# H263/review-based-recommender

Measured on NVIDIA B200. Metric: DeepCoNN fwd+bwd samples/sec, higher is better.
Workload: dtype bf16

## Files before the change

review-based-recommender_b200/csrc/conv_bwd_tc.cu:

```cuda
#include "rbr_common.cuh"
#include "tc_ptx.cuh"
#include "tma_util.cuh"

namespace rbr {

constexpr int CM_THREADS = 192;
constexpr int CM_STAGES_T = 3;
constexpr int CM_STAGES_W = 3;

struct CmatLayout {
    int64_t V, H, K, E, HJ, HJp, emb_pad, epad4;
    int64_t off_c32, off_chl, off_dw, total;
    int64_t n_chunks, hc;
};
struct CmatChunk { int64_t h_lo, h_n, col_lo, width, base; };
static CmatLayout cmat_layout(int64_t vocab, int64_t emb, int64_t filters, int64_t ksize) {
    CmatLayout l;
    l.V = vocab; l.H = filters; l.K = ksize; l.E = emb;
    l.HJ = filters * ksize;
    l.HJp = cmat_hjp(filters, ksize);
    l.emb_pad = rbr_emb_pad(emb);
    l.epad4 = round_up(emb, 4);
    int64_t off = 0;
    l.off_c32 = off; off += round_up(vocab * l.HJp * 4, 1024);
// ... 165 lines not shown
        hi.x = *reinterpret_cast<const uint32_t*>(&h01); hi.y = *reinterpret_cast<const uint32_t*>(&h23);
        lo.x = *reinterpret_cast<const uint32_t*>(&l01); lo.y = *reinterpret_cast<const uint32_t*>(&l23);
        __nv_bfloat16* row = chl + r * (2 * (int64_t)HJp);
        *reinterpret_cast<uint2*>(row + c) = hi;
        *reinterpret_cast<uint2*>(row + HJp + c) = lo;
    }
}

__device__ __forceinline__ uint64_t umma_desc_mn_sw128(uint32_t addr, uint32_t lbo, uint32_t sbo) {
    return (uint64_t)((addr >> 4) & 0x3FFFu) | ((uint64_t)((lbo >> 4) & 0x3FFFu) << 16) | ((uint64_t)((sbo >> 4) & 0x3FFFu) << 32) |
           (1ull << 46) | (2ull << 61);
}
__device__ __forceinline__ uint32_t umma_idesc_mn(int M, int N) { return umma_idesc(M, N) | (1u << 15) | (1u << 16); }

struct TableGemmArgs {
    int64_t vocab;
    int E, NT, nkb;
    int64_t padding_idx;
    float* table_grad;
    int overwrite;
    int tile0;
};

__global__ void __launch_bounds__(CM_THREADS, 2)
cmat_table_gemm_kernel(const __grid_constant__ CUtensorMap tmA, const __grid_constant__ CUtensorMap tmB, const TableGemmArgs a) {
    extern __shared__ uint8_t smem_raw[];
    const int warp = threadIdx.x >> 5, lane = threadIdx.x & 31;
    const uint32_t raw = smem_u32(smem_raw);
    const uint32_t sbase = (raw + 1023u) & ~1023u;
    uint8_t* smem = smem_raw + (sbase - raw);
    const int b_bytes = a.NT * 128;
    const int stage_bytes = 16384 + b_bytes;
    const uint32_t bars = sbase + CM_STAGES_T * stage_bytes;
    volatile uint32_t* tmem_slot = reinterpret_cast<volatile uint32_t*>(smem + CM_STAGES_T * stage_bytes + 8 * (2 * CM_STAGES_T + 1));
    const int m0 = ((int)blockIdx.x + a.tile0) * 128, n0 = blockIdx.y * a.NT;

    if (threadIdx.x == 0) {
        for (int i = 0; i < CM_STAGES_T; ++i) { mbar_init(bars + 8 * i, 1); mbar_init(bars + 8 * (CM_STAGES_T + i), 1); }
        mbar_init(bars + 16 * CM_STAGES_T, 1);
        fence_barrier_init();
    }
    if (warp == 1) tmem_alloc(smem_u32((const void*)tmem_slot), 256);
    tc_fence_before();
    __syncthreads();
    tc_fence_after();
    const uint32_t tmem_base = *tmem_slot;

    if (warp == 0) {
        if (elect_one()) {
            tma_prefetch_desc(&tmA);
            tma_prefetch_desc(&tmB);
            int stage = 0;
            uint32_t ph = 0;
            for (int kb = 0; kb < a.nkb; ++kb) {
                mbar_wait(bars + 8 * (CM_STAGES_T + stage), ph ^ 1);
                const uint32_t fb = bars + 8 * stage;
                mbar_expect_tx(fb, (uint32_t)stage_bytes);
                const uint32_t dst = sbase + stage * stage_bytes;
                tma_load_2d(dst, &tmA, kb * 64, m0, fb);
                tma_load_2d(dst + 16384, &tmB, kb * 64, n0, fb);
                if (++stage == CM_STAGES_T) { stage = 0; ph ^= 1; }
            }
        }
        __syncwarp();
    } else if (warp == 1) {
        const uint32_t idesc = umma_idesc(128, a.NT);
        int stage = 0;
        uint32_t ph = 0;
        for (int kb = 0; kb < a.nkb; ++kb) {
            mbar_wait(bars + 8 * stage, ph);
            tc_fence_after();
            if (elect_one()) {
                const uint32_t sa = sbase + stage * stage_bytes;
                const uint64_t ad = umma_desc_sw128(sa), bd = umma_desc_sw128(sa + 16384);
#pragma unroll
                for (int ks = 0; ks < 4; ++ks)
                    umma_bf16(tmem_base, ad + (uint64_t)(ks * 2), bd + (uint64_t)(ks * 2), idesc, (uint32_t)((kb | ks) != 0));
                umma_commit(bars + 8 * (CM_STAGES_T + stage));
                if (kb == a.nkb - 1) umma_commit(bars + 16 * CM_STAGES_T);
            }
            __syncwarp();
            if (++stage == CM_STAGES_T) { stage = 0; ph ^= 1; }
        }
    } else {
        const int quad = warp & 3;
        const int64_t row = (int64_t)m0 + quad * 32 + lane;
        const bool in_range = row < a.vocab;
        const bool pad_row = row == a.padding_idx;
        const bool live = in_range && (a.overwrite || !pad_row);
        const float keep = pad_row ? 0.f : 1.f;
        float* dst_row = a.table_grad + row * a.E;
        mbar_wait(bars + 16 * CM_STAGES_T, 0);
        tc_fence_after();
        const uint32_t taddr = tmem_base + ((uint32_t)(quad * 32) << 16);
        for (int c0 = 0; c0 < a.NT; c0 += 16) {
            uint32_t v[16];
            tmem_ld16(taddr + (uint32_t)c0, v);
            tmem_ld_wait();
            if (live) {
#pragma unroll
                for (int q = 0; q < 4; ++q) {
                    const int col = n0 + c0 + q * 4;
                    if (col + 3 < a.E) {
                        float4* p = reinterpret_cast<float4*>(dst_row + col);
                        float4 o = make_float4(0.f, 0.f, 0.f, 0.f);
                        if (!a.overwrite) o = *p;
                        o.x += keep * __uint_as_float(v[4 * q]); o.y += keep * __uint_as_float(v[4 * q + 1]);
                        o.z += keep * __uint_as_float(v[4 * q + 2]); o.w += keep * __uint_as_float(v[4 * q + 3]);
                        __stcs(p, o);
                    }
                }
            }
        }
    }
    tc_fence_before();
    __syncthreads();
    if (warp == 1) tmem_dealloc(tmem_base, 256);
}

struct WeightGemmArgs {
    int64_t vocab;
    int E, epad4, HJ, HJp, nch;
    int n_tb, ksplit;
    float* dw_hke;
};

__global__ void __launch_bounds__(CM_THREADS, 1)
cmat_weight_gemm_kernel(const __grid_constant__ CUtensorMap tmA, const __grid_constant__ CUtensorMap tmX, const WeightGemmArgs a) {
    extern __shared__ uint8_t smem_raw[];
    const int warp = threadIdx.x >> 5, lane = threadIdx.x & 31;
    const uint32_t raw = smem_u32(smem_raw);
    const uint32_t sbase = (raw + 1023u) & ~1023u;
    uint8_t* smem = smem_raw + (sbase - raw);
    const int stage_bytes = (2 + a.nch) * 8192;
    const uint32_t bars = sbase + CM_STAGES_W * stage_bytes;
    volatile uint32_t* tmem_slot = reinterpret_cast<volatile uint32_t*>(smem + CM_STAGES_W * stage_bytes + 8 * (2 * CM_STAGES_W + 1));
    const int m0 = blockIdx.x * 128;
    const int split = blockIdx.y;
    const int n_mine = (a.n_tb - split + a.ksplit - 1) / a.ksplit;
    const uint32_t tmem_cols = a.nch * 64 <= 256 ? 256u : 512u;

    if (threadIdx.x == 0) {
        for (int i = 0; i < CM_STAGES_W; ++i) { mbar_init(bars + 8 * i, 1); mbar_init(bars + 8 * (CM_STAGES_W + i), 1); }
        mbar_init(bars + 16 * CM_STAGES_W, 1);
        fence_barrier_init();
    }
    if (warp == 1) tmem_alloc(smem_u32((const void*)tmem_slot), tmem_cols);
    tc_fence_before();
    __syncthreads();
    tc_fence_after();
    const uint32_t tmem_base = *tmem_slot;

    if (n_mine > 0) {
        if (warp == 0) {
            if (elect_one()) {
                tma_prefetch_desc(&tmA);
                tma_prefetch_desc(&tmX);
                int stage = 0;
                uint32_t ph = 0;
                for (int i = 0; i < n_mine; ++i) {
                    const int row = (split + i * a.ksplit) * 64;
                    mbar_wait(bars + 8 * (CM_STAGES_W + stage), ph ^ 1);
                    const uint32_t fb = bars + 8 * stage;
                    mbar_expect_tx(fb, (uint32_t)stage_bytes);
                    const uint32_t dst = sbase + stage * stage_bytes;
                    tma_load_2d(dst, &tmA, m0, row, fb);
                    tma_load_2d(dst + 8192, &tmA, m0 + 64, row, fb);
                    for (int c = 0; c < a.nch; ++c) tma_load_2d(dst + 16384 + c * 8192, &tmX, c * 64, row, fb);
                    if (++stage == CM_STAGES_W) { stage = 0; ph ^= 1; }
                }
            }
            __syncwarp();
        } else if (warp == 1) {
            const int g0 = a.nch <= 4 ? a.nch : (a.nch + 1) / 2, g1 = a.nch - g0;
            const uint32_t idesc0 = umma_idesc_mn(128, g0 * 64), idesc1 = g1 ? umma_idesc_mn(128, g1 * 64) : 0u;
            int stage = 0;
            uint32_t ph = 0;
            for (int i = 0; i < n_mine; ++i) {
                mbar_wait(bars + 8 * stage, ph);
                tc_fence_after();
                if (elect_one()) {
                    const uint32_t sa = sbase + stage * stage_bytes, sb = sa + 16384;
#pragma unroll
                    for (int ks = 0; ks < 4; ++ks) {
                        const uint64_t ad = umma_desc_mn_sw128(sa + ks * 2048, 8192, 1024);
                        umma_bf16(tmem_base, ad, umma_desc_mn_sw128(sb + ks * 2048, 8192, 1024), idesc0, (uint32_t)((i | ks) != 0));
                        if (g1)
                            umma_bf16(tmem_base + (uint32_t)(g0 * 64), ad, umma_desc_mn_sw128(sb + g0 * 8192 + ks * 2048, 8192, 1024), idesc1,
                                      (uint32_t)((i | ks) != 0));
                    }
                    umma_commit(bars + 8 * (CM_STAGES_W + stage));
                    if (i == n_mine - 1) umma_commit(bars + 16 * CM_STAGES_W);
                }
                __syncwarp();
                if (++stage == CM_STAGES_W) { stage = 0; ph ^= 1; }
            }
        } else {
            const int quad = warp & 3;
            const int gm = m0 + quad * 32 + lane;
            const int hj = gm >= a.HJp ? gm - a.HJp : gm;
            const bool live = hj < a.HJ;
            float* dst_row = a.dw_hke + (int64_t)hj * a.epad4;
            mbar_wait(bars + 16 * CM_STAGES_W, 0);
            tc_fence_after();
            const uint32_t taddr = tmem_base + ((uint32_t)(quad * 32) << 16);
            for (int c0 = 0; c0 < a.nch * 64; c0 += 16) {
                uint32_t v[16];
                tmem_ld16(taddr + (uint32_t)c0, v);
                tmem_ld_wait();
                if (live) {
#pragma unroll
                    for (int q = 0; q < 4; ++q) {
                        const int col = c0 + q * 4;
                        if (col + 3 < a.E)
                            atomicAdd(reinterpret_cast<float4*>(dst_row + col),
                                      make_float4(__uint_as_float(v[4 * q]), __uint_as_float(v[4 * q + 1]), __uint_as_float(v[4 * q + 2]),
                                                  __uint_as_float(v[4 * q + 3])));
                    }
// ... 8 lines not shown

__global__ void cmat_unpack_kernel(float* __restrict__ dw_hke, int H, int E, int K, int epad4, float* __restrict__ wgrad) {
    const int64_t total = (int64_t)H * K * epad4;
    const int64_t stride = (int64_t)gridDim.x * blockDim.x;
    for (int64_t q = (int64_t)blockIdx.x * blockDim.x + threadIdx.x; q < total; q += stride) {
        const int e = (int)(q % epad4);
        const int hj = (int)(q / epad4);
        const float v = dw_hke[q];
        if (v != 0.f) {
            dw_hke[q] = 0.f;
            if (e < E) atomicAdd(wgrad + ((int64_t)(hj / K) * E + e) * K + (hj % K), v);
        }
    }
}

constexpr int CM_SMEM_T_MAX = 116 * 1024;
constexpr int CM_SMEM_W_MAX = 227 * 1024;
struct CmatSmem { int table, weight; };
static CmatSmem cmat_smem(int64_t emb) {
    int64_t NT, tiles;
    cmat_ntile(emb, &NT, &tiles);
    const int64_t nch = rbr_emb_pad(emb) / 64;
    CmatSmem s;
    s.table = CM_STAGES_T * (16384 + (int)NT * 128) + 8 * (2 * CM_STAGES_T + 1) + 16 + 1024;
    s.weight = CM_STAGES_W * (2 + (int)nch) * 8192 + 8 * (2 * CM_STAGES_W + 1) + 16 + 1024;
    return s;
}

static bool cmat_shape_ok(int64_t vocab, int64_t emb, int64_t filters, int64_t ksize) {
    if (vocab < 1 || vocab >= (1ll << 31) || emb < 4 || emb % 4 != 0 || emb > 512 || filters < 1 || ksize < 1 || ksize > 8) return false;
    if (filters > 1024) return false;
    const CmatSmem sm = cmat_smem(emb);
    if (sm.table > CM_SMEM_T_MAX || sm.weight > CM_SMEM_W_MAX) return false;
    const int64_t hjp = cmat_hjp(filters, ksize);
    if (hjp > 4096) return false;
    return vocab * hjp * 4 <= (3ll << 30);
}

}

using namespace rbr;

extern "C" int rbr_conv_bwd_cmat_supported(int64_t vocab, int64_t emb, int64_t filters, int64_t ksize) {
    return cmat_shape_ok(vocab, emb, filters, ksize) && tensor_map_encoder() != nullptr ? 1 : 0;
}
// ... 124 lines not shown
        for (int64_t c = (chunk < 0 ? 0 : chunk); c < (chunk < 0 ? l.n_chunks : chunk + 1); ++c) {
            const CmatChunk k = cmat_chunk(l, c);
            const int64_t total = vocab * (k.width / 4);
            int64_t blocks = (total + 255) / 256;
            if (blocks > 148 * 16) blocks = 148 * 16;
            cmat_split_kernel<<<(unsigned)blocks, 256, 0, s>>>(reinterpret_cast<const float4*>(c32 + k.base), vocab, (int)k.width, (int)k.col_lo,
                                                               (int)l.HJp, chl);
            RBR_LAUNCH_CHECK("cmat_split_kernel");
        }
    }
    if (what & 2) {
        RBR_REQUIRE(table_grad, RBR_EINVAL, "conv_bwd_cmat_finish: table part needs table_grad");
        RBR_REQUIRE((uintptr_t)table_grad % 16 == 0, RBR_EINVAL, "conv_bwd_cmat_finish: table_grad must be 16-byte aligned");
        CUtensorMap tmA, tmB;
        RBR_REQUIRE(make_tmap_bf16_2d(&tmA, chl, (uint64_t)(2 * l.HJp), (uint64_t)vocab, (uint64_t)(2 * l.HJp), 64, 128) &&
                        make_tmap_bf16_2d(&tmB, reinterpret_cast<const char*>(packed) + pl.off_wt2, (uint64_t)(2 * l.HJp),
                                          (uint64_t)(pl.NT * pl.n_tiles), (uint64_t)(2 * l.HJp), 64, (uint32_t)pl.NT),
                    RBR_ECUDA, "conv_bwd_cmat_finish: cuTensorMapEncodeTiled failed");
        TableGemmArgs a{};
        a.vocab = vocab; a.E = (int)emb; a.NT = (int)pl.NT; a.nkb = (int)(2 * l.HJp / 64); a.padding_idx = padding_idx;
        a.table_grad = table_grad;
        a.overwrite = (what & 8) ? 1 : 0;
        if (row_lo == 0 && row_hi == 0) row_hi = vocab;
        RBR_REQUIRE(row_lo >= 0 && row_lo < row_hi && row_hi <= vocab && row_lo % 128 == 0 && (row_hi % 128 == 0 || row_hi == vocab), RBR_EINVAL,
                    "conv_bwd_cmat_finish: the table row range must be cut on multiples of 128 rows");
        a.tile0 = (int)(row_lo / 128);
        const int smem = cmat_smem(emb).table;
        static bool attr = false;
        if (!attr) {
            RBR_CUDA(cudaFuncSetAttribute(cmat_table_gemm_kernel, cudaFuncAttributeMaxDynamicSharedMemorySize, CM_SMEM_T_MAX));
            attr = true;
        }
        RBR_REQUIRE(smem <= CM_SMEM_T_MAX, RBR_EUNSUPPORTED, "conv_bwd_cmat_finish: shared memory");
        dim3 grid((unsigned)((row_hi - row_lo + 127) / 128), (unsigned)pl.n_tiles);
        cmat_table_gemm_kernel<<<grid, CM_THREADS, smem, s>>>(tmA, tmB, a);
        RBR_LAUNCH_CHECK("cmat_table_gemm_kernel");
    }
    if (what & 4) {
        RBR_REQUIRE(weight_grad && shadow_bf16, RBR_EINVAL, "conv_bwd_cmat_finish: weight part needs weight_grad and the bf16 shadow table");
        CUtensorMap tmA, tmX;
        RBR_REQUIRE(make_tmap_bf16_2d(&tmA, chl, (uint64_t)(2 * l.HJp), (uint64_t)vocab, (uint64_t)(2 * l.HJp), 64, 64) &&
                        make_tmap_bf16_2d(&tmX, shadow_bf16, (uint64_t)l.emb_pad, (uint64_t)vocab, (uint64_t)l.emb_pad, 64, 64),
                    RBR_ECUDA, "conv_bwd_cmat_finish: cuTensorMapEncodeTiled failed");
        WeightGemmArgs a{};
        a.vocab = vocab; a.E = (int)emb; a.epad4 = (int)l.epad4; a.HJ = (int)l.HJ; a.HJp = (int)l.HJp; a.nch = (int)(l.emb_pad / 64);
        a.n_tb = (int)((vocab + 63) / 64);
        const int m_tiles = (int)(2 * l.HJp / 128);
        static int sms = 0;
        if (!sms) {
            int dev = 0;
            RBR_CUDA(cudaGetDevice(&dev));
            RBR_CUDA(cudaDeviceGetAttribute(&sms, cudaDevAttrMultiProcessorCount, dev));
        }
        a.ksplit = sms / m_tiles < 1 ? 1 : sms / m_tiles;
        if (a.ksplit > a.n_tb) a.ksplit = a.n_tb;
        a.dw_hke = dw;
        const int smem = cmat_smem(emb).weight;
        static bool attr = false;
        if (!attr) {
            RBR_CUDA(cudaFuncSetAttribute(cmat_weight_gemm_kernel, cudaFuncAttributeMaxDynamicSharedMemorySize, CM_SMEM_W_MAX));
            attr = true;
        }
        RBR_REQUIRE(smem <= CM_SMEM_W_MAX, RBR_EUNSUPPORTED, "conv_bwd_cmat_finish: shared memory");
        dim3 grid((unsigned)m_tiles, (unsigned)a.ksplit);
        cmat_weight_gemm_kernel<<<grid, CM_THREADS, smem, s>>>(tmA, tmX, a);
        RBR_LAUNCH_CHECK("cmat_weight_gemm_kernel");
        const int64_t tot = l.HJ * l.epad4;
        int blocks = (int)((tot + 255) / 256);
        if (blocks > 148 * 4) blocks = 148 * 4;
        cmat_unpack_kernel<<<blocks, 256, 0, s>>>(dw, (int)filters, (int)emb, (int)ksize, (int)l.epad4, weight_grad);
        RBR_LAUNCH_CHECK("cmat_unpack_kernel");
    }
    return RBR_OK;
}
```

review-based-recommender_b200/csrc/embed.cu:

```cuda
#include "rbr_common.cuh"
#include "token_sort.cuh"

namespace rbr {

template <int UNROLL>
__global__ void __launch_bounds__(256) gather_rows_v4_kernel(const float4* __restrict__ table, int64_t vocab, int e4,
                                                             const int64_t* __restrict__ ids, int64_t n_tokens,
                                                             float4* __restrict__ out) {
    const int64_t total = n_tokens * (int64_t)e4;
    const int64_t stride = (int64_t)gridDim.x * blockDim.x;
    int64_t q = (int64_t)blockIdx.x * blockDim.x + threadIdx.x;
    for (; q + (UNROLL - 1) * stride < total; q += UNROLL * stride) {
        float4 v[UNROLL];
        int64_t dst[UNROLL];
#pragma unroll
        for (int u = 0; u < UNROLL; ++u) {
            const int64_t p = q + u * stride;
            const int64_t tok = p / e4;
            const int c = (int)(p - tok * e4);
            const int64_t id = __ldg(ids + tok);
            dst[u] = p;
            if (id >= 0 && id < vocab) {
                v[u] = __ldg(table + id * e4 + c);
            } else {
// ... 119 lines not shown
#pragma unroll
        for (int j = 0; j < 8; ++j) f[j] = (c0 + j < emb) ? __ldg(src + j) : 0.f;
        uint4 pk;
        __nv_bfloat162 t;
        t = __floats2bfloat162_rn(f[0], f[1]); pk.x = *reinterpret_cast<uint32_t*>(&t);
        t = __floats2bfloat162_rn(f[2], f[3]); pk.y = *reinterpret_cast<uint32_t*>(&t);
        t = __floats2bfloat162_rn(f[4], f[5]); pk.z = *reinterpret_cast<uint32_t*>(&t);
        t = __floats2bfloat162_rn(f[6], f[7]); pk.w = *reinterpret_cast<uint32_t*>(&t);
        *reinterpret_cast<uint4*>(shadow + row * emb_pad + c0) = pk;
    }
}

__global__ void conv_pack_kernel(const float* __restrict__ w, int E, int H, int k, int Hpad4, int Epad4, int Epad16, int Npad, int Nb,
                                 int Npad2, int Nb2, float* __restrict__ keh, float* __restrict__ hke,
                                 __nv_bfloat16* __restrict__ umma, __nv_bfloat16* __restrict__ umma2, __nv_bfloat16* __restrict__ hke16,
                                 __nv_bfloat16* __restrict__ wt2, int HJp, int wt2_rows) {
    const int64_t n_keh = (int64_t)k * E * Hpad4;
    const int64_t n_hke = (int64_t)H * k * Epad4;
    const int64_t n_umma = (int64_t)k * Epad16 * Npad;
    const int64_t n_umma2 = (int64_t)k * Epad16 * Npad2;
    const int64_t n_wt2 = (int64_t)wt2_rows * 2 * HJp;
    const int64_t total = n_keh + n_hke + n_umma + n_umma2 + n_wt2;
    const int64_t stride = (int64_t)gridDim.x * blockDim.x;
    for (int64_t q = (int64_t)blockIdx.x * blockDim.x + threadIdx.x; q < total; q += stride) {
        if (q >= n_keh + n_hke + n_umma + n_umma2) {
            const int64_t r = q - (n_keh + n_hke + n_umma + n_umma2);
            const int e = (int)(r / (2 * HJp));
            int c = (int)(r - (int64_t)e * 2 * HJp);
            if (c >= HJp) c -= HJp;
            const int h = c / k, j = c - h * k;
            wt2[r] = __float2bfloat16_rn((e < E && h < H) ? w[((int64_t)h * E + e) * k + j] : 0.f);
        } else if (q < n_keh) {
            const int h = (int)(q % Hpad4);
            const int e = (int)((q / Hpad4) % E);
            const int j = (int)(q / ((int64_t)Hpad4 * E));
            keh[q] = (h < H) ? w[((int64_t)h * E + e) * k + j] : 0.f;
        } else if (q < n_keh + n_hke) {
            const int64_t r = q - n_keh;
            const int e = (int)(r % Epad4);
            const int j = (int)((r / Epad4) % k);
            const int h = (int)(r / ((int64_t)Epad4 * k));
            const float v = (e < E) ? w[((int64_t)h * E + e) * k + j] : 0.f;
            hke[r] = v;
            hke16[r] = __float2bfloat16_rn(v);
        } else if (q >= n_keh + n_hke + n_umma) {
            const int64_t r = q - n_keh - n_hke - n_umma;
// ... 113 lines not shown
}

extern "C" int64_t rbr_conv_pack_bytes(int64_t emb, int64_t filters, int64_t ksize) {
    return pack_layout(emb, filters, ksize).total;
}

extern "C" int rbr_conv_pack(const float* weight, int64_t emb, int64_t filters, int64_t ksize, void* packed, void* stream) {
    RBR_REQUIRE(weight && packed, RBR_EINVAL, "rbr_conv_pack: null pointer");
    RBR_REQUIRE(emb > 0 && filters > 0 && ksize > 0, RBR_EINVAL, "rbr_conv_pack: bad sizes");
    RBR_REQUIRE((uintptr_t)packed % 256 == 0, RBR_EINVAL, "rbr_conv_pack: packed buffer must be 256-byte aligned");
    const PackLayout p = pack_layout(emb, filters, ksize);
    char* base = reinterpret_cast<char*>(packed);
    RBR_CUDA(cudaMemsetAsync(base + p.off_zero, 0, (size_t)(p.off_umma2 - p.off_zero), as_stream(stream)));
    const int64_t npad2 = p.P2 * p.Nb2;
    const int64_t total = ksize * emb * p.Hpad4 + filters * ksize * p.Epad4 + ksize * p.Epad16 * (p.Npad + npad2) +
                          p.NT * p.n_tiles * 2 * p.HJp;
    conv_pack_kernel<<<grid_for(total, 256), 256, 0, as_stream(stream)>>>(
        weight, (int)emb, (int)filters, (int)ksize, (int)p.Hpad4, (int)p.Epad4, (int)p.Epad16, (int)p.Npad, (int)(p.Nb > 0 ? p.Nb : 1),
        (int)npad2, (int)(p.Nb2 > 0 ? p.Nb2 : 2), reinterpret_cast<float*>(base + p.off_keh), reinterpret_cast<float*>(base + p.off_hke),
        reinterpret_cast<__nv_bfloat16*>(base + p.off_umma), reinterpret_cast<__nv_bfloat16*>(base + p.off_umma2),
        reinterpret_cast<__nv_bfloat16*>(base + p.off_hke16), reinterpret_cast<__nv_bfloat16*>(base + p.off_wt2), (int)p.HJp,
        (int)(p.NT * p.n_tiles));
    RBR_LAUNCH_CHECK("conv_pack");
    return RBR_OK;
}

RBR_DEFINE_OOB_ACCESSOR(embed)
```

review-based-recommender_b200/csrc/rbr_common.cuh:

```cuda
#pragma once
#include <cuda_runtime.h>
#include <cuda_bf16.h>
#include <stdint.h>
#include <stdio.h>
#include <stdarg.h>

#include "../../include/rbr_b200.h"

namespace rbr {

void set_error(const char* fmt, ...);
int cuda_fail(cudaError_t e, const char* what);

#define RBR_REQUIRE(cond, code, ...)                    \
    do {                                                \
        if (!(cond)) {                                  \
            rbr::set_error(__VA_ARGS__);                \
            return (code);                              \
        }                                               \
    } while (0)

#define RBR_CUDA(call)                                                   \
    do {                                                                 \
        cudaError_t e__ = (call);                                        \
// ... 26 lines not shown
void tc_pass_split(int64_t E, int64_t H, int64_t K, int64_t* P, int64_t* Nb);
void tc2_pass_split(int64_t E, int64_t H, int64_t K, int64_t* P, int64_t* Nb);
struct PackLayout {
    int64_t E, H, k;
    int64_t P, Nb;
    int64_t P2, Nb2;
    int64_t off_umma2;
    int64_t off_hke16;
    int64_t Hpad4;
    int64_t Epad4;
    int64_t Epad16;
    int64_t Npad;
    int64_t off_keh, off_hke, off_umma, off_zero, total;
    int64_t HJp;
    int64_t NT, n_tiles;
    int64_t off_wt2;
};
__host__ __device__ inline int64_t round_up(int64_t x, int64_t m) { return (x + m - 1) / m * m; }
inline int64_t cmat_hjp(int64_t H, int64_t k) { return round_up(H * k, 64); }
inline void cmat_ntile(int64_t E, int64_t* NT, int64_t* tiles) {
    *NT = E > 128 ? 160 : round_up(E, 16);
    *tiles = (E + *NT - 1) / *NT;
}
inline PackLayout pack_layout(int64_t E, int64_t H, int64_t k) {
    PackLayout p;
    p.E = E; p.H = H; p.k = k;
    p.Hpad4 = round_up(H, 4);
    p.Epad4 = round_up(E, 4);
    p.Epad16 = round_up(E, 16);
    tc_pass_split(E, H, k, &p.P, &p.Nb);
    p.Npad = p.P * p.Nb;
    p.off_keh = 0;
    int64_t b = k * E * p.Hpad4 * 4;
    p.off_hke = round_up(b, 256);
    b = p.off_hke + H * k * p.Epad4 * 4;
    p.off_umma = round_up(b, 256);
    b = p.off_umma + k * p.Epad16 * p.Npad * 2;
    p.off_zero = round_up(b, 256);
    b = p.off_zero + round_up(E, 64) * 2 + 256;
    p.off_umma2 = round_up(b, 256);
    tc2_pass_split(E, H, k, &p.P2, &p.Nb2);
    b = p.off_umma2 + k * p.Epad16 * p.P2 * p.Nb2 * 2;
    p.off_hke16 = round_up(b, 256);
    b = p.off_hke16 + H * k * p.Epad4 * 2;
    p.off_wt2 = round_up(b, 1024);
    p.HJp = cmat_hjp(H, k);
    cmat_ntile(E, &p.NT, &p.n_tiles);
    b = p.off_wt2 + p.NT * p.n_tiles * 2 * p.HJp * 2;
    p.total = round_up(b, 256);
    return p;
}

__device__ __forceinline__ float warp_sum(float v) {
#pragma unroll
    for (int o = 16; o > 0; o >>= 1) v += __shfl_xor_sync(0xffffffffu, v, o);
    return v;
}
__device__ __forceinline__ float warp_max(float v) {
#pragma unroll
    for (int o = 16; o > 0; o >>= 1) v = fmaxf(v, __shfl_xor_sync(0xffffffffu, v, o));
    return v;
}

// ... 36 lines not shown
```

review-based-recommender_b200/csrc/tc_ptx.cuh:

```cuda
#pragma once
#include "rbr_common.cuh"

namespace rbr {

__device__ __forceinline__ uint32_t smem_u32(const void* p) { return (uint32_t)__cvta_generic_to_shared(p); }

__device__ __forceinline__ void mbar_init(uint32_t bar, uint32_t count) {
    asm volatile("mbarrier.init.shared::cta.b64 [%0], %1;" ::"r"(bar), "r"(count));
}
__device__ __forceinline__ void mbar_arrive(uint32_t bar) {
    asm volatile("mbarrier.arrive.shared::cta.b64 _, [%0];" ::"r"(bar) : "memory");
}
__device__ __forceinline__ void mbar_expect_tx(uint32_t bar, uint32_t bytes) {
    asm volatile("mbarrier.arrive.expect_tx.shared::cta.b64 _, [%0], %1;" ::"r"(bar), "r"(bytes) : "memory");
}
__device__ __forceinline__ bool mbar_try_wait(uint32_t bar, uint32_t parity) {
    uint32_t ok;
    asm volatile(
        "{\n\t.reg .pred p;\n\t"
        "mbarrier.try_wait.parity.shared::cta.b64 p, [%1], %2;\n\t"
        "selp.u32 %0, 1, 0, p;\n\t}"
        : "=r"(ok)
        : "r"(bar), "r"(parity)
        : "memory");
// ... 55 lines not shown
}
__device__ __forceinline__ uint32_t umma_idesc(int M, int N) {
    return (1u << 4) | (1u << 7) | (1u << 10) | ((uint32_t)(N >> 3) << 17) | ((uint32_t)(M >> 4) << 24);
}
__device__ __forceinline__ void umma_bf16(uint32_t tmem_d, uint64_t adesc, uint64_t bdesc, uint32_t idesc, uint32_t accumulate) {
    asm volatile(
        "{\n\t.reg .pred p;\n\t"
        "setp.ne.b32 p, %4, 0;\n\t"
        "tcgen05.mma.cta_group::1.kind::f16 [%0], %1, %2, %3, p;\n\t}" ::"r"(tmem_d),
        "l"(adesc), "l"(bdesc), "r"(idesc), "r"(accumulate)
        : "memory");
}
__device__ __forceinline__ void umma_commit(uint32_t bar) {
    asm volatile("tcgen05.commit.cta_group::1.mbarrier::arrive::one.shared::cluster.b64 [%0];" ::"r"(bar) : "memory");
}
__device__ __forceinline__ void tmem_ld16(uint32_t taddr, uint32_t (&v)[16]) {
    asm volatile(
        "tcgen05.ld.sync.aligned.32x32b.x16.b32 {%0,%1,%2,%3,%4,%5,%6,%7,%8,%9,%10,%11,%12,%13,%14,%15}, [%16];"
        : "=r"(v[0]), "=r"(v[1]), "=r"(v[2]), "=r"(v[3]), "=r"(v[4]), "=r"(v[5]), "=r"(v[6]), "=r"(v[7]), "=r"(v[8]), "=r"(v[9]),
          "=r"(v[10]), "=r"(v[11]), "=r"(v[12]), "=r"(v[13]), "=r"(v[14]), "=r"(v[15])
        : "r"(taddr)
        : "memory");
}
__device__ __forceinline__ bool elect_one() {
    uint32_t pred;
    asm volatile(
        "{\n\t.reg .pred p;\n\t"
        "elect.sync _|p, 0xffffffff;\n\t"
        "selp.u32 %0, 1, 0, p;\n\t}"
        : "=r"(pred));
// ... 26 lines not shown
    }
#pragma unroll
    for (int i = 0; i < 16; ++i) {
        const uint32_t b = __ballot_sync(0xffffffffu, (FULL || mine) && (int)v[i] == r[i]);
        if ((lane & 15) == i) { keep_v = (uint32_t)r[i]; keep_b = b; }
    }
}



__device__ __forceinline__ uint32_t cluster_ctarank() {
    uint32_t r;
    asm volatile("mov.u32 %0, %%cluster_ctarank;" : "=r"(r));
    return r;
}
__device__ __forceinline__ void cluster_sync_all() {
    asm volatile("barrier.cluster.arrive.release.aligned;\n\tbarrier.cluster.wait.acquire.aligned;" ::: "memory");
}
__device__ __forceinline__ void mbar_arrive_cluster(uint32_t bar, uint32_t cta) {
    asm volatile(
        "{\n\t.reg .b32 ra;\n\t"
        "mapa.shared::cluster.u32 ra, %0, %1;\n\t"
        "mbarrier.arrive.shared::cluster.b64 _, [ra];\n\t}" ::"r"(bar), "r"(cta)
        : "memory");
}
__device__ __forceinline__ void tmem_alloc2(uint32_t slot_smem, uint32_t cols) {
    asm volatile("tcgen05.alloc.cta_group::2.sync.aligned.shared::cta.b32 [%0], %1;" ::"r"(slot_smem), "r"(cols) : "memory");
    asm volatile("tcgen05.relinquish_alloc_permit.cta_group::2.sync.aligned;" ::: "memory");
}
__device__ __forceinline__ void tmem_dealloc2(uint32_t taddr, uint32_t cols) {
// ... 32 lines not shown
```

review-based-recommender_b200/csrc/tma_util.cuh:

```cuda
#pragma once
#include <cuda.h>

#include "rbr_common.cuh"

namespace rbr {

typedef CUresult (*EncodeTiledFn)(CUtensorMap*, CUtensorMapDataType, cuuint32_t, void*, const cuuint64_t*, const cuuint64_t*,
                                  const cuuint32_t*, const cuuint32_t*, CUtensorMapInterleave, CUtensorMapSwizzle,
                                  CUtensorMapL2promotion, CUtensorMapFloatOOBfill);

inline EncodeTiledFn tensor_map_encoder() {
    static EncodeTiledFn fn = nullptr;
    static bool tried = false;
    if (!tried) {
        tried = true;
        void* f = nullptr;
        cudaDriverEntryPointQueryResult q;
        if (cudaGetDriverEntryPoint("cuTensorMapEncodeTiled", &f, cudaEnableDefault, &q) == cudaSuccess &&
            q == cudaDriverEntryPointSuccess)
            fn = reinterpret_cast<EncodeTiledFn>(f);
        else
            (void)cudaGetLastError();
    }
    return fn;
}

inline bool make_tmap_bf16_2d(CUtensorMap* tm, const void* base, uint64_t cols, uint64_t rows, uint64_t pitch_elems,
                              uint32_t box_cols, uint32_t box_rows) {
    EncodeTiledFn enc = tensor_map_encoder();
    if (!enc) return false;
    cuuint64_t gdim[2] = {(cuuint64_t)cols, (cuuint64_t)rows};
    cuuint64_t gstr[1] = {(cuuint64_t)pitch_elems * 2};
    cuuint32_t box[2] = {box_cols, box_rows};
    cuuint32_t estr[2] = {1, 1};
    return enc(tm, CU_TENSOR_MAP_DATA_TYPE_BFLOAT16, 2, const_cast<void*>(base), gdim, gstr, box, estr, CU_TENSOR_MAP_INTERLEAVE_NONE,
               CU_TENSOR_MAP_SWIZZLE_128B, CU_TENSOR_MAP_L2_PROMOTION_L2_256B, CU_TENSOR_MAP_FLOAT_OOB_FILL_NONE) == CUDA_SUCCESS;
}

__device__ __forceinline__ void tma_load_2d(uint32_t dst, const void* tmap, int col, int row, uint32_t bar) {
    asm volatile(
        "cp.async.bulk.tensor.2d.shared::cluster.global.tile.mbarrier::complete_tx::bytes [%0], [%1, {%2, %3}], [%4];" ::"r"(dst),
        "l"(tmap), "r"(col), "r"(row), "r"(bar)
        : "memory");
}

}
```

Measured before the change: 5.348 million.

## Multicast table-GEMM A tiles across cluster, TMA-store epilogue, split hi/lo weights

Restructures the embedding-table gradient GEMM. The hi and lo halves of the split-bf16 C matrix now load as two A boxes sharing one B tile, multicast across a CTA cluster, and the packed weight copy holding the duplicated B becomes a single non-duplicated one. The epilogue stages results in swizzled shared memory and writes them out with TMA store or reduce-add bulk ops instead of per-thread float4 read-modify-write. The weight GEMM loads hi and lo through separate tensor maps and accumulates both into the same TMEM. This cuts global traffic and scattered stores, at the cost of cluster synchronisation, fewer table pipeline stages and a lower supported maximum embedding size.

```diff
diff --git a/review-based-recommender_b200/csrc/conv_bwd_tc.cu b/review-based-recommender_b200/csrc/conv_bwd_tc.cu
--- a/review-based-recommender_b200/csrc/conv_bwd_tc.cu
+++ b/review-based-recommender_b200/csrc/conv_bwd_tc.cu
@@ -5,8 +5,7 @@
 namespace rbr {
 
 constexpr int CM_THREADS = 192;
-constexpr int CM_STAGES_T = 3;
-constexpr int CM_STAGES_W = 3;
+constexpr int CM_STAGES_T = 2;
 
 struct CmatLayout {
     int64_t V, H, K, E, HJ, HJp, emb_pad, epad4;
@@ -203,35 +202,38 @@
 __device__ __forceinline__ uint32_t umma_idesc_mn(int M, int N) { return umma_idesc(M, N) | (1u << 15) | (1u << 16); }
 
 struct TableGemmArgs {
-    int64_t vocab;
-    int E, NT, nkb;
+    int NT, HJp, nkb;
+    int nbox;
     int64_t padding_idx;
-    float* table_grad;
     int overwrite;
     int tile0;
 };
 
 __global__ void __launch_bounds__(CM_THREADS, 2)
-cmat_table_gemm_kernel(const __grid_constant__ CUtensorMap tmA, const __grid_constant__ CUtensorMap tmB, const TableGemmArgs a) {
+cmat_table_gemm_kernel(const __grid_constant__ CUtensorMap tmA, const __grid_constant__ CUtensorMap tmB, const __grid_constant__ CUtensorMap tmOut,
+                       const TableGemmArgs a) {
     extern __shared__ uint8_t smem_raw[];
     const int warp = threadIdx.x >> 5, lane = threadIdx.x & 31;
     const uint32_t raw = smem_u32(smem_raw);
     const uint32_t sbase = (raw + 1023u) & ~1023u;
     uint8_t* smem = smem_raw + (sbase - raw);
     const int b_bytes = a.NT * 128;
-    const int stage_bytes = 16384 + b_bytes;
+    const int stage_bytes = 2 * 16384 + b_bytes;
     const uint32_t bars = sbase + CM_STAGES_T * stage_bytes;
     volatile uint32_t* tmem_slot = reinterpret_cast<volatile uint32_t*>(smem + CM_STAGES_T * stage_bytes + 8 * (2 * CM_STAGES_T + 1));
     const int m0 = ((int)blockIdx.x + a.tile0) * 128, n0 = blockIdx.y * a.NT;
+    const int ncta = (int)cluster_nctarank();
+    const int rank = (int)cluster_ctarank();
+    const uint16_t cluster_mask = (uint16_t)((1u << ncta) - 1u);
 
     if (threadIdx.x == 0) {
-        for (int i = 0; i < CM_STAGES_T; ++i) { mbar_init(bars + 8 * i, 1); mbar_init(bars + 8 * (CM_STAGES_T + i), 1); }
+        for (int i = 0; i < CM_STAGES_T; ++i) { mbar_init(bars + 8 * i, 1); mbar_init(bars + 8 * (CM_STAGES_T + i), (uint32_t)ncta); }
         mbar_init(bars + 16 * CM_STAGES_T, 1);
         fence_barrier_init();
     }
     if (warp == 1) tmem_alloc(smem_u32((const void*)tmem_slot), 256);
     tc_fence_before();
-    __syncthreads();
+    cluster_sync_all();
     tc_fence_after();
     const uint32_t tmem_base = *tmem_slot;
 
@@ -246,8 +248,15 @@
                 const uint32_t fb = bars + 8 * stage;
                 mbar_expect_tx(fb, (uint32_t)stage_bytes);
                 const uint32_t dst = sbase + stage * stage_bytes;
-                tma_load_2d(dst, &tmA, kb * 64, m0, fb);
-                tma_load_2d(dst + 16384, &tmB, kb * 64, n0, fb);
+                for (int b = rank; b < 2; b += ncta) {
+                    if (ncta == 1) tma_load_2d(dst + b * 16384, &tmA, b * a.HJp + kb * 64, m0, fb);
+                    else tma_load_2d_mc(dst + b * 16384, &tmA, b * a.HJp + kb * 64, m0, fb, cluster_mask);
+                }
+                tma_load_2d(dst + 2 * 16384, &tmB, kb * 64, n0, fb);
+                if (++stage == CM_STAGES_T) { stage = 0; ph ^= 1; }
+            }
+            for (int i = 0; i < CM_STAGES_T; ++i) {
+                mbar_wait(bars + 8 * (CM_STAGES_T + stage), ph ^ 1);
                 if (++stage == CM_STAGES_T) { stage = 0; ph ^= 1; }
             }
         }
@@ -261,11 +270,16 @@
             tc_fence_after();
             if (elect_one()) {
                 const uint32_t sa = sbase + stage * stage_bytes;
-                const uint64_t ad = umma_desc_sw128(sa), bd = umma_desc_sw128(sa + 16384);
-#pragma unroll
-                for (int ks = 0; ks < 4; ++ks)
-                    umma_bf16(tmem_base, ad + (uint64_t)(ks * 2), bd + (uint64_t)(ks * 2), idesc, (uint32_t)((kb | ks) != 0));
-                umma_commit(bars + 8 * (CM_STAGES_T + stage));
+                const uint64_t bd = umma_desc_sw128(sa + 2 * 16384);
+#pragma unroll
+                for (int b = 0; b < 2; ++b) {
+                    const uint64_t ad = umma_desc_sw128(sa + b * 16384);
+#pragma unroll
+                    for (int ks = 0; ks < 4; ++ks)
+                        umma_bf16(tmem_base, ad + (uint64_t)(ks * 2), bd + (uint64_t)(ks * 2), idesc, (uint32_t)((kb | b | ks) != 0));
+                }
+                if (ncta == 1) umma_commit(bars + 8 * (CM_STAGES_T + stage));
+                else umma_commit_mc(bars + 8 * (CM_STAGES_T + stage), cluster_mask);
                 if (kb == a.nkb - 1) umma_commit(bars + 16 * CM_STAGES_T);
             }
             __syncwarp();
@@ -273,65 +287,70 @@
         }
     } else {
         const int quad = warp & 3;
-        const int64_t row = (int64_t)m0 + quad * 32 + lane;
-        const bool in_range = row < a.vocab;
-        const bool pad_row = row == a.padding_idx;
-        const bool live = in_range && (a.overwrite || !pad_row);
-        const float keep = pad_row ? 0.f : 1.f;
-        float* dst_row = a.table_grad + row * a.E;
+        const int row0 = m0 + quad * 32;
+        const bool pad_row = (int64_t)(row0 + lane) == a.padding_idx;
+        const uint32_t out = sbase + (uint32_t)(quad * a.nbox) * 4096u;
         mbar_wait(bars + 16 * CM_STAGES_T, 0);
         tc_fence_after();
         const uint32_t taddr = tmem_base + ((uint32_t)(quad * 32) << 16);
-        for (int c0 = 0; c0 < a.NT; c0 += 16) {
+        for (int c0 = 0; c0 < a.nbox * 32; c0 += 16) {
             uint32_t v[16];
             tmem_ld16(taddr + (uint32_t)c0, v);
             tmem_ld_wait();
-            if (live) {
-#pragma unroll
-                for (int q = 0; q < 4; ++q) {
-                    const int col = n0 + c0 + q * 4;
-                    if (col + 3 < a.E) {
-                        float4* p = reinterpret_cast<float4*>(dst_row + col);
-                        float4 o = make_float4(0.f, 0.f, 0.f, 0.f);
-                        if (!a.overwrite) o = *p;
-                        o.x += keep * __uint_as_float(v[4 * q]); o.y += keep * __uint_as_float(v[4 * q + 1]);
-                        o.z += keep * __uint_as_float(v[4 * q + 2]); o.w += keep * __uint_as_float(v[4 * q + 3]);
-                        __stcs(p, o);
-                    }
-                }
-            }
-        }
+            const uint32_t line = out + (uint32_t)(c0 >> 5) * 4096u + (uint32_t)lane * 128u;
+#pragma unroll
+            for (int q = 0; q < 4; ++q) {
+                const uint32_t chunk = (uint32_t)(((c0 & 31) >> 2) + q);
+                st_shared_v4(line + ((chunk ^ (uint32_t)(lane & 7)) << 4), pad_row ? 0u : v[4 * q], pad_row ? 0u : v[4 * q + 1],
+                             pad_row ? 0u : v[4 * q + 2], pad_row ? 0u : v[4 * q + 3]);
+            }
+        }
+        fence_proxy_async();
+        __syncwarp();
+        if (lane == 0) {
+            const uint64_t policy = l2_policy_evict_first();
+            for (int b = 0; b < a.nbox; ++b) {
+                if (a.overwrite) tma_store_2d(&tmOut, out + (uint32_t)b * 4096u, n0 + b * 32, row0, policy);
+                else tma_reduce_add_2d(&tmOut, out + (uint32_t)b * 4096u, n0 + b * 32, row0, policy);
+            }
+            bulk_commit_group();
+            bulk_wait_group_read0();
+        }
+        __syncwarp();
     }
     tc_fence_before();
-    __syncthreads();
+    cluster_sync_all();
     if (warp == 1) tmem_dealloc(tmem_base, 256);
 }
 
 struct WeightGemmArgs {
     int64_t vocab;
-    int E, epad4, HJ, HJp, nch;
+    int E, epad4, HJ, nch;
+    int stages;
     int n_tb, ksplit;
     float* dw_hke;
 };
 
 __global__ void __launch_bounds__(CM_THREADS, 1)
-cmat_weight_gemm_kernel(const __grid_constant__ CUtensorMap tmA, const __grid_constant__ CUtensorMap tmX, const WeightGemmArgs a) {
+cmat_weight_gemm_kernel(const __grid_constant__ CUtensorMap tmHi, const __grid_constant__ CUtensorMap tmLo, const __grid_constant__ CUtensorMap tmX,
+                        const WeightGemmArgs a) {
     extern __shared__ uint8_t smem_raw[];
     const int warp = threadIdx.x >> 5, lane = threadIdx.x & 31;
     const uint32_t raw = smem_u32(smem_raw);
     const uint32_t sbase = (raw + 1023u) & ~1023u;
     uint8_t* smem = smem_raw + (sbase - raw);
-    const int stage_bytes = (2 + a.nch) * 8192;
-    const uint32_t bars = sbase + CM_STAGES_W * stage_bytes;
-    volatile uint32_t* tmem_slot = reinterpret_cast<volatile uint32_t*>(smem + CM_STAGES_W * stage_bytes + 8 * (2 * CM_STAGES_W + 1));
+    const int S = a.stages;
+    const int stage_bytes = (4 + a.nch) * 8192;
+    const uint32_t bars = sbase + S * stage_bytes;
+    volatile uint32_t* tmem_slot = reinterpret_cast<volatile uint32_t*>(smem + S * stage_bytes + 8 * (2 * S + 1));
     const int m0 = blockIdx.x * 128;
     const int split = blockIdx.y;
     const int n_mine = (a.n_tb - split + a.ksplit - 1) / a.ksplit;
     const uint32_t tmem_cols = a.nch * 64 <= 256 ? 256u : 512u;
 
     if (threadIdx.x == 0) {
-        for (int i = 0; i < CM_STAGES_W; ++i) { mbar_init(bars + 8 * i, 1); mbar_init(bars + 8 * (CM_STAGES_W + i), 1); }
-        mbar_init(bars + 16 * CM_STAGES_W, 1);
+        for (int i = 0; i < S; ++i) { mbar_init(bars + 8 * i, 1); mbar_init(bars + 8 * (S + i), 1); }
+        mbar_init(bars + 16 * S, 1);
         fence_barrier_init();
     }
     if (warp == 1) tmem_alloc(smem_u32((const void*)tmem_slot), tmem_cols);
@@ -343,20 +362,23 @@
     if (n_mine > 0) {
         if (warp == 0) {
             if (elect_one()) {
-                tma_prefetch_desc(&tmA);
+                tma_prefetch_desc(&tmHi);
+                tma_prefetch_desc(&tmLo);
                 tma_prefetch_desc(&tmX);
                 int stage = 0;
                 uint32_t ph = 0;
                 for (int i = 0; i < n_mine; ++i) {
                     const int row = (split + i * a.ksplit) * 64;
-                    mbar_wait(bars + 8 * (CM_STAGES_W + stage), ph ^ 1);
+                    mbar_wait(bars + 8 * (S + stage), ph ^ 1);
                     const uint32_t fb = bars + 8 * stage;
                     mbar_expect_tx(fb, (uint32_t)stage_bytes);
                     const uint32_t dst = sbase + stage * stage_bytes;
-                    tma_load_2d(dst, &tmA, m0, row, fb);
-                    tma_load_2d(dst + 8192, &tmA, m0 + 64, row, fb);
-                    for (int c = 0; c < a.nch; ++c) tma_load_2d(dst + 16384 + c * 8192, &tmX, c * 64, row, fb);
-                    if (++stage == CM_STAGES_W) { stage = 0; ph ^= 1; }
+                    tma_load_2d(dst, &tmHi, m0, row, fb);
+                    tma_load_2d(dst + 8192, &tmHi, m0 + 64, row, fb);
+                    tma_load_2d(dst + 2 * 8192, &tmLo, m0, row, fb);
+                    tma_load_2d(dst + 3 * 8192, &tmLo, m0 + 64, row, fb);
+                    for (int c = 0; c < a.nch; ++c) tma_load_2d(dst + (4 + c) * 8192, &tmX, c * 64, row, fb);
+                    if (++stage == S) { stage = 0; ph ^= 1; }
                 }
             }
             __syncwarp();
@@ -369,28 +391,31 @@
                 mbar_wait(bars + 8 * stage, ph);
                 tc_fence_after();
                 if (elect_one()) {
-                    const uint32_t sa = sbase + stage * stage_bytes, sb = sa + 16384;
+                    const uint32_t sa = sbase + stage * stage_bytes, sb = sa + 4 * 8192;
 #pragma unroll
                     for (int ks = 0; ks < 4; ++ks) {
-                        const uint64_t ad = umma_desc_mn_sw128(sa + ks * 2048, 8192, 1024);
-                        umma_bf16(tmem_base, ad, umma_desc_mn_sw128(sb + ks * 2048, 8192, 1024), idesc0, (uint32_t)((i | ks) != 0));
-                        if (g1)
-                            umma_bf16(tmem_base + (uint32_t)(g0 * 64), ad, umma_desc_mn_sw128(sb + g0 * 8192 + ks * 2048, 8192, 1024), idesc1,
-                                      (uint32_t)((i | ks) != 0));
+                        const uint64_t bd0 = umma_desc_mn_sw128(sb + ks * 2048, 8192, 1024);
+                        const uint64_t bd1 = umma_desc_mn_sw128(sb + g0 * 8192 + ks * 2048, 8192, 1024);
+#pragma unroll
+                        for (int h = 0; h < 2; ++h) {
+                            const uint64_t ad = umma_desc_mn_sw128(sa + h * 16384 + ks * 2048, 8192, 1024);
+                            const uint32_t acc = (uint32_t)((i | ks | h) != 0);
+                            umma_bf16(tmem_base, ad, bd0, idesc0, acc);
+                            if (g1) umma_bf16(tmem_base + (uint32_t)(g0 * 64), ad, bd1, idesc1, acc);
+                        }
                     }
-                    umma_commit(bars + 8 * (CM_STAGES_W + stage));
-                    if (i == n_mine - 1) umma_commit(bars + 16 * CM_STAGES_W);
+                    umma_commit(bars + 8 * (S + stage));
+                    if (i == n_mine - 1) umma_commit(bars + 16 * S);
                 }
                 __syncwarp();
-                if (++stage == CM_STAGES_W) { stage = 0; ph ^= 1; }
+                if (++stage == S) { stage = 0; ph ^= 1; }
             }
         } else {
             const int quad = warp & 3;
-            const int gm = m0 + quad * 32 + lane;
-            const int hj = gm >= a.HJp ? gm - a.HJp : gm;
+            const int hj = m0 + quad * 32 + lane;
             const bool live = hj < a.HJ;
             float* dst_row = a.dw_hke + (int64_t)hj * a.epad4;
-            mbar_wait(bars + 16 * CM_STAGES_W, 0);
+            mbar_wait(bars + 16 * S, 0);
             tc_fence_after();
             const uint32_t taddr = tmem_base + ((uint32_t)(quad * 32) << 16);
             for (int c0 = 0; c0 < a.nch * 64; c0 += 16) {
@@ -429,21 +454,23 @@
     }
 }
 
-constexpr int CM_SMEM_T_MAX = 116 * 1024;
+constexpr int CM_SMEM_T_MAX = 112 * 1024;
 constexpr int CM_SMEM_W_MAX = 227 * 1024;
+static int cmat_w_smem(int64_t nch, int stages) { return stages * (4 + (int)nch) * 8192 + 8 * (2 * stages + 1) + 16 + 1024; }
+static int cmat_w_stages(int64_t nch) { return cmat_w_smem(nch, 3) <= CM_SMEM_W_MAX ? 3 : 2; }
 struct CmatSmem { int table, weight; };
 static CmatSmem cmat_smem(int64_t emb) {
     int64_t NT, tiles;
     cmat_ntile(emb, &NT, &tiles);
     const int64_t nch = rbr_emb_pad(emb) / 64;
     CmatSmem s;
-    s.table = CM_STAGES_T * (16384 + (int)NT * 128) + 8 * (2 * CM_STAGES_T + 1) + 16 + 1024;
-    s.weight = CM_STAGES_W * (2 + (int)nch) * 8192 + 8 * (2 * CM_STAGES_W + 1) + 16 + 1024;
+    s.table = CM_STAGES_T * (2 * 16384 + (int)NT * 128) + 8 * (2 * CM_STAGES_T + 1) + 16 + 1024;
+    s.weight = cmat_w_smem(nch, cmat_w_stages(nch));
     return s;
 }
 
 static bool cmat_shape_ok(int64_t vocab, int64_t emb, int64_t filters, int64_t ksize) {
-    if (vocab < 1 || vocab >= (1ll << 31) || emb < 4 || emb % 4 != 0 || emb > 512 || filters < 1 || ksize < 1 || ksize > 8) return false;
+    if (vocab < 1 || vocab >= (1ll << 31) || emb < 4 || emb % 4 != 0 || emb > 448 || filters < 1 || ksize < 1 || ksize > 8) return false;
     if (filters > 1024) return false;
     const CmatSmem sm = cmat_smem(emb);
     if (sm.table > CM_SMEM_T_MAX || sm.weight > CM_SMEM_W_MAX) return false;
@@ -598,12 +625,14 @@
         RBR_REQUIRE((uintptr_t)table_grad % 16 == 0, RBR_EINVAL, "conv_bwd_cmat_finish: table_grad must be 16-byte aligned");
         CUtensorMap tmA, tmB;
         RBR_REQUIRE(make_tmap_bf16_2d(&tmA, chl, (uint64_t)(2 * l.HJp), (uint64_t)vocab, (uint64_t)(2 * l.HJp), 64, 128) &&
-                        make_tmap_bf16_2d(&tmB, reinterpret_cast<const char*>(packed) + pl.off_wt2, (uint64_t)(2 * l.HJp),
-                                          (uint64_t)(pl.NT * pl.n_tiles), (uint64_t)(2 * l.HJp), 64, (uint32_t)pl.NT),
+                        make_tmap_bf16_2d(&tmB, reinterpret_cast<const char*>(packed) + pl.off_wt, (uint64_t)l.HJp,
+                                          (uint64_t)(pl.NT * pl.n_tiles), (uint64_t)l.HJp, 64, (uint32_t)pl.NT),
                     RBR_ECUDA, "conv_bwd_cmat_finish: cuTensorMapEncodeTiled failed");
+        CUtensorMap tmOut;
+        RBR_REQUIRE(make_tmap_f32_2d(&tmOut, table_grad, (uint64_t)emb, (uint64_t)vocab, (uint64_t)emb, 32, 32), RBR_ECUDA,
+                    "conv_bwd_cmat_finish: cuTensorMapEncodeTiled failed");
         TableGemmArgs a{};
-        a.vocab = vocab; a.E = (int)emb; a.NT = (int)pl.NT; a.nkb = (int)(2 * l.HJp / 64); a.padding_idx = padding_idx;
-        a.table_grad = table_grad;
+        a.NT = (int)pl.NT; a.HJp = (int)l.HJp; a.nkb = (int)(l.HJp / 64); a.nbox = (int)((pl.NT + 31) / 32); a.padding_idx = padding_idx;
         a.overwrite = (what & 8) ? 1 : 0;
         if (row_lo == 0 && row_hi == 0) row_hi = vocab;
         RBR_REQUIRE(row_lo >= 0 && row_lo < row_hi && row_hi <= vocab && row_lo % 128 == 0 && (row_hi % 128 == 0 || row_hi == vocab), RBR_EINVAL,
@@ -616,20 +645,31 @@
             attr = true;
         }
         RBR_REQUIRE(smem <= CM_SMEM_T_MAX, RBR_EUNSUPPORTED, "conv_bwd_cmat_finish: shared memory");
-        dim3 grid((unsigned)((row_hi - row_lo + 127) / 128), (unsigned)pl.n_tiles);
-        cmat_table_gemm_kernel<<<grid, CM_THREADS, smem, s>>>(tmA, tmB, a);
+        cudaLaunchConfig_t cfg{};
+        cfg.gridDim = dim3((unsigned)((row_hi - row_lo + 127) / 128), (unsigned)pl.n_tiles);
+        cfg.blockDim = dim3(CM_THREADS);
+        cfg.dynamicSmemBytes = (size_t)smem;
+        cfg.stream = s;
+        cudaLaunchAttribute attr_cl[1];
+        attr_cl[0].id = cudaLaunchAttributeClusterDimension;
+        attr_cl[0].val.clusterDim.x = 1; attr_cl[0].val.clusterDim.y = (unsigned)pl.n_tiles; attr_cl[0].val.clusterDim.z = 1;
+        cfg.attrs = attr_cl;
+        cfg.numAttrs = 1;
+        RBR_CUDA(cudaLaunchKernelEx(&cfg, cmat_table_gemm_kernel, tmA, tmB, tmOut, a));
         RBR_LAUNCH_CHECK("cmat_table_gemm_kernel");
     }
     if (what & 4) {
         RBR_REQUIRE(weight_grad && shadow_bf16, RBR_EINVAL, "conv_bwd_cmat_finish: weight part needs weight_grad and the bf16 shadow table");
-        CUtensorMap tmA, tmX;
-        RBR_REQUIRE(make_tmap_bf16_2d(&tmA, chl, (uint64_t)(2 * l.HJp), (uint64_t)vocab, (uint64_t)(2 * l.HJp), 64, 64) &&
+        CUtensorMap tmHi, tmLo, tmX;
+        RBR_REQUIRE(make_tmap_bf16_2d(&tmHi, chl, (uint64_t)l.HJp, (uint64_t)vocab, (uint64_t)(2 * l.HJp), 64, 64) &&
+                        make_tmap_bf16_2d(&tmLo, chl + l.HJp, (uint64_t)l.HJp, (uint64_t)vocab, (uint64_t)(2 * l.HJp), 64, 64) &&
                         make_tmap_bf16_2d(&tmX, shadow_bf16, (uint64_t)l.emb_pad, (uint64_t)vocab, (uint64_t)l.emb_pad, 64, 64),
                     RBR_ECUDA, "conv_bwd_cmat_finish: cuTensorMapEncodeTiled failed");
         WeightGemmArgs a{};
-        a.vocab = vocab; a.E = (int)emb; a.epad4 = (int)l.epad4; a.HJ = (int)l.HJ; a.HJp = (int)l.HJp; a.nch = (int)(l.emb_pad / 64);
+        a.vocab = vocab; a.E = (int)emb; a.epad4 = (int)l.epad4; a.HJ = (int)l.HJ; a.nch = (int)(l.emb_pad / 64);
+        a.stages = cmat_w_stages(a.nch);
         a.n_tb = (int)((vocab + 63) / 64);
-        const int m_tiles = (int)(2 * l.HJp / 128);
+        const int m_tiles = (int)((l.HJp + 127) / 128);
         static int sms = 0;
         if (!sms) {
             int dev = 0;
@@ -647,7 +687,7 @@
         }
         RBR_REQUIRE(smem <= CM_SMEM_W_MAX, RBR_EUNSUPPORTED, "conv_bwd_cmat_finish: shared memory");
         dim3 grid((unsigned)m_tiles, (unsigned)a.ksplit);
-        cmat_weight_gemm_kernel<<<grid, CM_THREADS, smem, s>>>(tmA, tmX, a);
+        cmat_weight_gemm_kernel<<<grid, CM_THREADS, smem, s>>>(tmHi, tmLo, tmX, a);
         RBR_LAUNCH_CHECK("cmat_weight_gemm_kernel");
         const int64_t tot = l.HJ * l.epad4;
         int blocks = (int)((tot + 255) / 256);
diff --git a/review-based-recommender_b200/csrc/embed.cu b/review-based-recommender_b200/csrc/embed.cu
--- a/review-based-recommender_b200/csrc/embed.cu
+++ b/review-based-recommender_b200/csrc/embed.cu
@@ -157,22 +157,21 @@
 __global__ void conv_pack_kernel(const float* __restrict__ w, int E, int H, int k, int Hpad4, int Epad4, int Epad16, int Npad, int Nb,
                                  int Npad2, int Nb2, float* __restrict__ keh, float* __restrict__ hke,
                                  __nv_bfloat16* __restrict__ umma, __nv_bfloat16* __restrict__ umma2, __nv_bfloat16* __restrict__ hke16,
-                                 __nv_bfloat16* __restrict__ wt2, int HJp, int wt2_rows) {
+                                 __nv_bfloat16* __restrict__ wt, int HJp, int wt_rows) {
     const int64_t n_keh = (int64_t)k * E * Hpad4;
     const int64_t n_hke = (int64_t)H * k * Epad4;
     const int64_t n_umma = (int64_t)k * Epad16 * Npad;
     const int64_t n_umma2 = (int64_t)k * Epad16 * Npad2;
-    const int64_t n_wt2 = (int64_t)wt2_rows * 2 * HJp;
-    const int64_t total = n_keh + n_hke + n_umma + n_umma2 + n_wt2;
+    const int64_t n_wt = (int64_t)wt_rows * HJp;
+    const int64_t total = n_keh + n_hke + n_umma + n_umma2 + n_wt;
     const int64_t stride = (int64_t)gridDim.x * blockDim.x;
     for (int64_t q = (int64_t)blockIdx.x * blockDim.x + threadIdx.x; q < total; q += stride) {
         if (q >= n_keh + n_hke + n_umma + n_umma2) {
             const int64_t r = q - (n_keh + n_hke + n_umma + n_umma2);
-            const int e = (int)(r / (2 * HJp));
-            int c = (int)(r - (int64_t)e * 2 * HJp);
-            if (c >= HJp) c -= HJp;
+            const int e = (int)(r / HJp);
+            const int c = (int)(r - (int64_t)e * HJp);
             const int h = c / k, j = c - h * k;
-            wt2[r] = __float2bfloat16_rn((e < E && h < H) ? w[((int64_t)h * E + e) * k + j] : 0.f);
+            wt[r] = __float2bfloat16_rn((e < E && h < H) ? w[((int64_t)h * E + e) * k + j] : 0.f);
         } else if (q < n_keh) {
             const int h = (int)(q % Hpad4);
             const int e = (int)((q / Hpad4) % E);
@@ -316,12 +315,12 @@
     RBR_CUDA(cudaMemsetAsync(base + p.off_zero, 0, (size_t)(p.off_umma2 - p.off_zero), as_stream(stream)));
     const int64_t npad2 = p.P2 * p.Nb2;
     const int64_t total = ksize * emb * p.Hpad4 + filters * ksize * p.Epad4 + ksize * p.Epad16 * (p.Npad + npad2) +
-                          p.NT * p.n_tiles * 2 * p.HJp;
+                          p.NT * p.n_tiles * p.HJp;
     conv_pack_kernel<<<grid_for(total, 256), 256, 0, as_stream(stream)>>>(
         weight, (int)emb, (int)filters, (int)ksize, (int)p.Hpad4, (int)p.Epad4, (int)p.Epad16, (int)p.Npad, (int)(p.Nb > 0 ? p.Nb : 1),
         (int)npad2, (int)(p.Nb2 > 0 ? p.Nb2 : 2), reinterpret_cast<float*>(base + p.off_keh), reinterpret_cast<float*>(base + p.off_hke),
         reinterpret_cast<__nv_bfloat16*>(base + p.off_umma), reinterpret_cast<__nv_bfloat16*>(base + p.off_umma2),
-        reinterpret_cast<__nv_bfloat16*>(base + p.off_hke16), reinterpret_cast<__nv_bfloat16*>(base + p.off_wt2), (int)p.HJp,
+        reinterpret_cast<__nv_bfloat16*>(base + p.off_hke16), reinterpret_cast<__nv_bfloat16*>(base + p.off_wt), (int)p.HJp,
         (int)(p.NT * p.n_tiles));
     RBR_LAUNCH_CHECK("conv_pack");
     return RBR_OK;
diff --git a/review-based-recommender_b200/csrc/rbr_common.cuh b/review-based-recommender_b200/csrc/rbr_common.cuh
--- a/review-based-recommender_b200/csrc/rbr_common.cuh
+++ b/review-based-recommender_b200/csrc/rbr_common.cuh
@@ -64,7 +64,7 @@
     int64_t off_keh, off_hke, off_umma, off_zero, total;
     int64_t HJp;
     int64_t NT, n_tiles;
-    int64_t off_wt2;
+    int64_t off_wt;
 };
 __host__ __device__ inline int64_t round_up(int64_t x, int64_t m) { return (x + m - 1) / m * m; }
 inline int64_t cmat_hjp(int64_t H, int64_t k) { return round_up(H * k, 64); }
@@ -93,10 +93,10 @@
     b = p.off_umma2 + k * p.Epad16 * p.P2 * p.Nb2 * 2;
     p.off_hke16 = round_up(b, 256);
     b = p.off_hke16 + H * k * p.Epad4 * 2;
-    p.off_wt2 = round_up(b, 1024);
+    p.off_wt = round_up(b, 1024);
     p.HJp = cmat_hjp(H, k);
     cmat_ntile(E, &p.NT, &p.n_tiles);
-    b = p.off_wt2 + p.NT * p.n_tiles * 2 * p.HJp * 2;
+    b = p.off_wt + p.NT * p.n_tiles * p.HJp * 2;
     p.total = round_up(b, 256);
     return p;
 }
diff --git a/review-based-recommender_b200/csrc/tc_ptx.cuh b/review-based-recommender_b200/csrc/tc_ptx.cuh
--- a/review-based-recommender_b200/csrc/tc_ptx.cuh
+++ b/review-based-recommender_b200/csrc/tc_ptx.cuh
@@ -93,6 +93,11 @@
 __device__ __forceinline__ void umma_commit(uint32_t bar) {
     asm volatile("tcgen05.commit.cta_group::1.mbarrier::arrive::one.shared::cluster.b64 [%0];" ::"r"(bar) : "memory");
 }
+__device__ __forceinline__ void umma_commit_mc(uint32_t bar, uint16_t cta_mask) {
+    asm volatile("tcgen05.commit.cta_group::1.mbarrier::arrive::one.shared::cluster.multicast::cluster.b64 [%0], %1;" ::"r"(bar),
+                 "h"(cta_mask)
+                 : "memory");
+}
 __device__ __forceinline__ void tmem_ld16(uint32_t taddr, uint32_t (&v)[16]) {
     asm volatile(
         "tcgen05.ld.sync.aligned.32x32b.x16.b32 {%0,%1,%2,%3,%4,%5,%6,%7,%8,%9,%10,%11,%12,%13,%14,%15}, [%16];"
@@ -149,6 +154,11 @@
     asm volatile("mov.u32 %0, %%cluster_ctarank;" : "=r"(r));
     return r;
 }
+__device__ __forceinline__ uint32_t cluster_nctarank() {
+    uint32_t r;
+    asm volatile("mov.u32 %0, %%cluster_nctarank;" : "=r"(r));
+    return r;
+}
 __device__ __forceinline__ void cluster_sync_all() {
     asm volatile("barrier.cluster.arrive.release.aligned;\n\tbarrier.cluster.wait.acquire.aligned;" ::: "memory");
 }
diff --git a/review-based-recommender_b200/csrc/tma_util.cuh b/review-based-recommender_b200/csrc/tma_util.cuh
--- a/review-based-recommender_b200/csrc/tma_util.cuh
+++ b/review-based-recommender_b200/csrc/tma_util.cuh
@@ -37,6 +37,18 @@
                CU_TENSOR_MAP_SWIZZLE_128B, CU_TENSOR_MAP_L2_PROMOTION_L2_256B, CU_TENSOR_MAP_FLOAT_OOB_FILL_NONE) == CUDA_SUCCESS;
 }
 
+inline bool make_tmap_f32_2d(CUtensorMap* tm, const void* base, uint64_t cols, uint64_t rows, uint64_t pitch_elems,
+                             uint32_t box_cols, uint32_t box_rows) {
+    EncodeTiledFn enc = tensor_map_encoder();
+    if (!enc) return false;
+    cuuint64_t gdim[2] = {(cuuint64_t)cols, (cuuint64_t)rows};
+    cuuint64_t gstr[1] = {(cuuint64_t)pitch_elems * 4};
+    cuuint32_t box[2] = {box_cols, box_rows};
+    cuuint32_t estr[2] = {1, 1};
+    return enc(tm, CU_TENSOR_MAP_DATA_TYPE_FLOAT32, 2, const_cast<void*>(base), gdim, gstr, box, estr, CU_TENSOR_MAP_INTERLEAVE_NONE,
+               CU_TENSOR_MAP_SWIZZLE_128B, CU_TENSOR_MAP_L2_PROMOTION_L2_256B, CU_TENSOR_MAP_FLOAT_OOB_FILL_NONE) == CUDA_SUCCESS;
+}
+
 __device__ __forceinline__ void tma_load_2d(uint32_t dst, const void* tmap, int col, int row, uint32_t bar) {
     asm volatile(
         "cp.async.bulk.tensor.2d.shared::cluster.global.tile.mbarrier::complete_tx::bytes [%0], [%1, {%2, %3}], [%4];" ::"r"(dst),
@@ -44,4 +56,32 @@
         : "memory");
 }
 
+__device__ __forceinline__ void tma_load_2d_mc(uint32_t dst, const void* tmap, int col, int row, uint32_t bar, uint16_t cta_mask) {
+    asm volatile(
+        "cp.async.bulk.tensor.2d.shared::cluster.global.tile.mbarrier::complete_tx::bytes.multicast::cluster [%0], [%1, {%2, %3}], [%4], %5;" ::"r"(dst),
+        "l"(tmap), "r"(col), "r"(row), "r"(bar), "h"(cta_mask)
+        : "memory");
 }
+
+__device__ __forceinline__ void tma_store_2d(const void* tmap, uint32_t src, int col, int row, uint64_t policy) {
+    asm volatile("cp.async.bulk.tensor.2d.global.shared::cta.bulk_group.L2::cache_hint [%0, {%2, %3}], [%1], %4;" ::"l"(tmap), "r"(src),
+                 "r"(col), "r"(row), "l"(policy)
+                 : "memory");
+}
+__device__ __forceinline__ void tma_reduce_add_2d(const void* tmap, uint32_t src, int col, int row, uint64_t policy) {
+    asm volatile("cp.reduce.async.bulk.tensor.2d.global.shared::cta.add.tile.bulk_group.L2::cache_hint [%0, {%2, %3}], [%1], %4;" ::"l"(tmap),
+                 "r"(src), "r"(col), "r"(row), "l"(policy)
+                 : "memory");
+}
+__device__ __forceinline__ void bulk_commit_group() { asm volatile("cp.async.bulk.commit_group;" ::: "memory"); }
+__device__ __forceinline__ void bulk_wait_group_read0() { asm volatile("cp.async.bulk.wait_group.read 0;" ::: "memory"); }
+__device__ __forceinline__ uint64_t l2_policy_evict_first() {
+    uint64_t p;
+    asm volatile("createpolicy.fractional.L2::evict_first.b64 %0, 1.0;" : "=l"(p));
+    return p;
+}
+__device__ __forceinline__ void st_shared_v4(uint32_t addr, uint32_t x, uint32_t y, uint32_t z, uint32_t w) {
+    asm volatile("st.shared.v4.b32 [%0], {%1, %2, %3, %4};" ::"r"(addr), "r"(x), "r"(y), "r"(z), "r"(w) : "memory");
+}
+
+}
```

New measurement: 5.494 million (median of 6 runs). +2.7%, better.
